# theori-io/nrsc5

Measured on AMD Instinct MI355X. Metric: IQ MS/s demod+decoded, higher is better.
Workload: dtype exact float32 half-band (== int16 Q15) / f32 OFDM + sync / int32 Viterbi metrics

## Files before the change

include/nrsc5hip.h:

```cpp
#ifndef NRSC5HIP_H_
#define NRSC5HIP_H_

#include <stddef.h>
#include <stdint.h>

#ifdef __cplusplus
extern "C" {
#endif

#define NRSC5HIP_OK            0
#define NRSC5HIP_EINVAL       (-1)
#define NRSC5HIP_ENOMEM       (-2)
#define NRSC5HIP_EHIP         (-3)
#define NRSC5HIP_EOVERFLOW    (-4)

#define NRSC5HIP_P1_FRAME_BITS   146176
#define NRSC5HIP_P1_FRAME_WORDS  4568
#define NRSC5HIP_PIDS_FRAME_BITS 80

enum { NRSC5HIP_MODE_FM = 0, NRSC5HIP_MODE_AM = 1 };
#define NRSC5HIP_AM_P1_FRAME_BITS  3750
#define NRSC5HIP_AM_P3_BITS_MA1    24000
#define NRSC5HIP_AM_P3_BITS_MA3    30000

// ... 33 lines not shown
    int32_t bc_decoded;
    uint32_t pids[3];
    uint32_t sis;
} nrsc5hip_record;

typedef struct nrsc5hip_config {
    int device;
    int max_streams;
    long long q15_capacity;
    int record_capacity;
    int p1_slots;
    int p1_async;
    int l2_feedback;
    int am_enable;
    int batch_zero_copy;
    int l2_index;
} nrsc5hip_config;

typedef struct nrsc5hip_engine nrsc5hip_engine;

int nrsc5hip_engine_create(const nrsc5hip_config *cfg, nrsc5hip_engine **out);
void nrsc5hip_engine_destroy(nrsc5hip_engine *e);
const char *nrsc5hip_last_error(void);
const char *nrsc5hip_source_sha(void);
void *nrsc5hip_engine_hip_stream(nrsc5hip_engine *e);

int nrsc5hip_device_count(int *n);
int nrsc5hip_device_upload(int device, const void *host, size_t nbytes, void **dev_out);
int nrsc5hip_device_free(int device, void *dev);

int nrsc5hip_push_cu8(nrsc5hip_engine *e, int stream, const uint8_t *iq, uint32_t nbytes);
int nrsc5hip_push_cs16(nrsc5hip_engine *e, int stream, const int16_t *iq, uint32_t n);
int nrsc5hip_stream_reset(nrsc5hip_engine *e, int stream);
#define NRSC5HIP_ABI_VERSION 16
int nrsc5hip_abi_version(void);
int nrsc5hip_stream_fresh(nrsc5hip_engine *e, int stream);
int nrsc5hip_stream_set_mode(nrsc5hip_engine *e, int stream, int mode);
int nrsc5hip_force_resync(nrsc5hip_engine *e, int stream);
long long nrsc5hip_bytes_to_next_block(nrsc5hip_engine *e, int stream, int cu8);
int nrsc5hip_drain_ready(nrsc5hip_engine *e, int stream, nrsc5hip_record *out, int max, int *n_out);
int nrsc5hip_stream_set_manual_step(nrsc5hip_engine *e, int stream, int on);
int nrsc5hip_stream_step(nrsc5hip_engine *e, int stream);
int nrsc5hip_stream_step_ahead(nrsc5hip_engine *e, int stream, int *submitted);

int nrsc5hip_batch_append_cu8(nrsc5hip_engine *e, int nstreams, const int *stream_ids,
                              const uint8_t *dev_iq, long long stride_bytes, const uint32_t *nbytes);
int nrsc5hip_batch_append_cs16(nrsc5hip_engine *e, int nstreams, const int *stream_ids,
                               const int16_t *dev_iq, long long stride_elems, const uint32_t *nelems);
#define NRSC5HIP_TRIM_RETAIN_MAX    ((8LL * 16 + 1) * 71280)
#define NRSC5HIP_TRIM_RETAIN_MAX_AM ((8LL * 8 + 1) * 8910)
int nrsc5hip_batch_trim(nrsc5hip_engine *e, int nstreams, const int *stream_ids, long long *retained);
int nrsc5hip_batch_process(nrsc5hip_engine *e, int nstreams, const int *stream_ids, int max_steps, int *steps_done);

int nrsc5hip_drain(nrsc5hip_engine *e, int stream, nrsc5hip_record *out, int max, int *n_out);
int nrsc5hip_p1_frame_packed(nrsc5hip_engine *e, int stream, int slot, uint32_t *words );
int nrsc5hip_p1_frame_bits(nrsc5hip_engine *e, int stream, int slot, uint8_t *bits );
int nrsc5hip_px_frame_bits(nrsc5hip_engine *e, int stream, int slot, int channel, int nbits, uint8_t *bits);
int nrsc5hip_batch_fetch_px(nrsc5hip_engine *e, int nstreams, const int *stream_ids, uint32_t *frames);
int nrsc5hip_am_frame_bits(nrsc5hip_engine *e, int stream, int slot, int which, int nbits, uint8_t *bits);
int nrsc5hip_batch_fetch(nrsc5hip_engine *e, int nstreams, const int *stream_ids, nrsc5hip_record *records,
                         int max_records, int *counts, uint32_t *frames);
int nrsc5hip_batch_fetch_view(nrsc5hip_engine *e, int nstreams, const nrsc5hip_record **records, int *counts, const uint32_t **frames);
void nrsc5hip_unpack_bits(const uint32_t *words, int nbits, uint8_t *bits);

#define NRSC5HIP_L2_MAX_PDUS     16
#define NRSC5HIP_L2_MAX_PACKETS  64
#define NRSC5HIP_L2_MAX_BYTES    18269
// ... 131 lines not shown
int nrsc5hip_stage_aas(nrsc5hip_aas *a, int nstreams, const int *targets, const uint8_t *const *packets, const int *nbytes,
                       nrsc5hip_aas_event_cb cb, void *opaque);
int nrsc5hip_stage_aas_frames(nrsc5hip_aas *a, nrsc5hip_psd *psd, nrsc5hip_engine *e, int nstreams, const int *targets, const uint8_t *const *bits,
                              const int *nbits, const int *nframes, const int *lcs, const int *reset_at, nrsc5hip_aas_event_cb cb, void *opaque);
int nrsc5hip_aas_debug_arena(nrsc5hip_aas *a, long long bytes);

int nrsc5hip_stage_halfband_fm_cu8(nrsc5hip_engine *e, const uint8_t *iq, uint32_t nbytes, int16_t *out );
int nrsc5hip_stage_fft2048(nrsc5hip_engine *e, const float *in , float *out, int n);
int nrsc5hip_stage_viterbi_k7(nrsc5hip_engine *e, const int8_t *soft , int len, int nframes,
                              uint8_t *bits );
int nrsc5hip_stage_first_header(nrsc5hip_engine *e, const uint8_t *bits, int nbits, int nframes, int threads, int *ok);
int nrsc5hip_stage_viterbi_k9(nrsc5hip_engine *e, const int8_t *soft , int len, int nframes,
                              const unsigned gens[3], uint8_t *bits );
int nrsc5hip_stage_selftest(nrsc5hip_engine *e, int *failures);
enum { NRSC5HIP_MATH_REF_SINCOSF = 0, NRSC5HIP_MATH_REF_ATAN2F, NRSC5HIP_MATH_FAST_SINCOS, NRSC5HIP_MATH_FAST_SINCOS_REDUCED,
       NRSC5HIP_MATH_FAST_ATAN2, NRSC5HIP_MATH_SMALL_COS_SIN, NRSC5HIP_MATH_SMALL_ATAN };
int nrsc5hip_stage_math(nrsc5hip_engine *e, int fn, const void *a, const void *b, long long n, void *out0, void *out1);
enum { NRSC5HIP_HB_ACQ = 0, NRSC5HIP_HB_SYM128, NRSC5HIP_HB_SYM256 };
int nrsc5hip_stage_halfband_raw(nrsc5hip_engine *e, int form, const uint8_t *iq, size_t nbytes, int lead, long long a0, long long n,
                                int16_t *out, uint32_t *probe);
int nrsc5hip_stage_p1_deint(nrsc5hip_engine *e, const int8_t *pm, uint32_t *out);
int nrsc5hip_stage_p1_frame(nrsc5hip_engine *e, const int8_t *soft, int walk, uint8_t *bits, int *errors);
int nrsc5hip_stage_pids(nrsc5hip_engine *e, const int8_t *pm, int bc, int8_t *coded, uint8_t *bits, int *crc_ok);
int nrsc5hip_stage_px_interleave(nrsc5hip_engine *e, int len, int npairs, const int8_t *pairs, int8_t *out, int *ready);
int nrsc5hip_stage_am_deinterleave(nrsc5hip_engine *e, int psmi, int nframes, const uint8_t *sym, int8_t *v1, int8_t *v3);
enum { NRSC5HIP_CODE_E1 = 1, NRSC5HIP_CODE_E2 = 2 };
int nrsc5hip_stage_am_epilogue(nrsc5hip_engine *e, const int8_t *soft, const uint8_t *bits, int len, int code, int threads, int *errors,
                               uint8_t *bits_out, uint32_t *words_out);
int nrsc5hip_stage_acquire(nrsc5hip_engine *e, int n, const int16_t *win, const int16_t *hist, const int *state, const int *fill,
                           int16_t *filt, float *sums, int *samperr, float *peak, int16_t *hist_out);
int nrsc5hip_stage_acquire_raw(nrsc5hip_engine *e, int n, const uint8_t *iq, long long nbytes, const long long *rd, const int16_t *hist, const int *state,
                               int16_t *acq_win, int16_t *filt, float *sums, int *samperr, float *peak, int16_t *hist_out);
int nrsc5hip_stage_am_acquire(nrsc5hip_engine *e, const int16_t *win, const int16_t *hist, int state, int fill, int *samperr, float *peak, int16_t *hist_out);
int nrsc5hip_stage_viterbi_k7_debug(nrsc5hip_engine *e, const int8_t *soft, int len, uint8_t *bits, unsigned long long *dec_out);
int nrsc5hip_stage_viterbi_bench(nrsc5hip_engine *e, int len, int nframes, int phases, int reps, float *ms_per_launch);
int nrsc5hip_stage_viterbi_k9_bench(nrsc5hip_engine *e, int len, int nframes, int phases, int reps, float *ms_per_launch);
enum {
    NRSC5HIP_TUNE_DECODE_STREAMS = 0,
    NRSC5HIP_TUNE_AM_DECODE_STREAMS,
    NRSC5HIP_TUNE_VERDICT_LAG,
    NRSC5HIP_TUNE_SYNC_PHASES,
    NRSC5HIP_TUNE_FWD_SEGMENTS
    , NRSC5HIP_TUNE_FWD_WARM
    , NRSC5HIP_TUNE_AM_SEGMENTS
    , NRSC5HIP_TUNE_DECODE_CUS
    , NRSC5HIP_TUNE_DECODE_PRIORITY
    , NRSC5HIP_TUNE_AM_WARM
    , NRSC5HIP_TUNE_MIXFFT_SYMS
    , NRSC5HIP_TUNE_DEFER_WAIT
    , NRSC5HIP_TUNE_TRACEBACK_WALK
    , NRSC5HIP_TUNE_SYNC_LANES
    , NRSC5HIP_TUNE_DIRECT_DECIMATE
    , NRSC5HIP_TUNE_EARLY_FLUSH_KB
    , NRSC5HIP_TUNE_SEAM_PREPARE
    , NRSC5HIP_TUNE_NCO_EXACT
    , NRSC5HIP_TUNE_FLOW_MIN
    , NRSC5HIP_TUNE_LOOP_EXACT
    , NRSC5HIP_TUNE_HOST_CAPTURE
    , NRSC5HIP_TUNE_FOLD_REPORT
};
void nrsc5hip_debug_seam_totals(double out[8], int reset);
void nrsc5hip_debug_seam_counts(double out[6], int reset);
int nrsc5hip_debug_poison_results(nrsc5hip_engine *e);
int nrsc5hip_debug_fwd_stats(nrsc5hip_engine *e, int stats[2]);
int nrsc5hip_debug_flow_stats(nrsc5hip_engine *e, long long stats[2]);
int nrsc5hip_debug_host_capture_stats(nrsc5hip_engine *e, long long stats[5]);
// ... 95 lines not shown
```

nrsc5_amd/csrc/engine_stage.hip:

```cpp
#include <algorithm>
#include <cmath>
#include "engine_internal.h"

extern "C" void nrsc5hip_debug_seam_totals(double out[8], int reset)
{
    for (int k = 0; k < 8; k++) { if (out) out[k] = g_seam[k]; if (reset) g_seam[k] = 0; }
}
extern "C" void nrsc5hip_debug_seam_counts(double out[6], int reset)
{
    for (int k = 0; k < 6; k++) { if (out) out[k] = g_seam[8 + k]; if (reset) g_seam[8 + k] = 0; }
}

extern "C" int nrsc5hip_stage_l2_index(nrsc5hip_engine *e, const uint8_t *bits, int nbits, int nframes, nrsc5hip_l2_frame *out, uint8_t *pdu_bytes, long long stride)
{
    ON_ENGINE_DEVICE(e);
    if (!e || !bits || !out || nbits < 1 || nframes < 1) FAIL(NRSC5HIP_EINVAL, "bad argument");
    const int words = (nbits + 31) / 32;
    std::vector<uint32_t> w((size_t)words * nframes, 0u);
    for (int f = 0; f < nframes; f++)
        for (int i = 0; i < nbits; i++) w[(size_t)f * words + (i >> 5)] |= (uint32_t)(bits[(size_t)f * nbits + i] & 1u) << (i & 31);
    DevTmp tw;
    HIPCHK(hipMalloc(&tw.p, w.size() * sizeof(uint32_t)));
    uint32_t *dw = (uint32_t *)tw.p;
    HIPCHK(hipMemcpy(dw, w.data(), w.size() * sizeof(uint32_t), hipMemcpyHostToDevice));
// ... 490 lines not shown
    std::vector<unsigned> counts((size_t)n, (unsigned)nbytes);
    HIPCHK(hipMemcpy(e->nbytes_dev, counts.data(), counts.size() * sizeof(unsigned), hipMemcpyHostToDevice));
    launch_attach_raw(e->db, n, nullptr, (const uint8_t *)draw.p, nbytes, e->nbytes_dev, e->main);
    HIPCHK(hipGetLastError());
    HIPCHK(hipStreamSynchronize(e->main));
    for (int s = 0; s < n; s++) {
        POKE(e->db.state + s, StreamState, rd, rd[s]);
        if ((rc = acq_poke(e, s, hist + (size_t)s * 62, state[s]))) return rc;
    }
    return acq_run_fm(e, n, acq_win, filt, sums, samperr, peak, hist_out);
}

extern "C" int nrsc5hip_stage_am_acquire(nrsc5hip_engine *e, const int16_t *win, const int16_t *hist, int state, int fill, int *samperr, float *peak, int16_t *hist_out)
{
    ON_ENGINE_DEVICE(e);
    if (!win || !hist || !samperr || !peak || !hist_out) FAIL(NRSC5HIP_EINVAL, "null argument");
    if (!e->db.am) FAIL(NRSC5HIP_EINVAL, "engine was created without am_enable");
    int rc = acq_check_common(e, 1, &state, MODE_AM, AM_WIN); if (rc) return rc;
    if (fill < 0 || fill > AM_WIN) FAIL(NRSC5HIP_EINVAL, "fill %d: 0 .. %d samples", fill, AM_WIN);
    if ((rc = nrsc5hip_stream_fresh(e, 0))) return rc;
    DevBuffers db = e->db;
    db.l2_ring = nullptr; db.l2_px_ring = nullptr; db.l2_am_ring = nullptr; db.p1_mirror = nullptr;
    HIPCHK(hipMemcpy(db.q15, win, (size_t)AM_WIN * sizeof(c16), hipMemcpyHostToDevice));
    POKE(db.state, StreamState, wr, (long long)fill);
    if ((rc = acq_poke(e, 0, hist, state))) return rc;
    HIPCHK(hipMemsetAsync(db.counters, 0, 4 * sizeof(int), e->main));
    launch_am_step(e->tb, db, 1, nullptr, e->main, e->cfg.l2_feedback, e->cfg.p1_async ? 0 : -1, 0, 0);
    HIPCHK(hipGetLastError());
    HIPCHK(hipStreamSynchronize(e->main));
    if ((rc = acq_peek(e, 0, samperr, peak, hist_out))) return rc;
    return nrsc5hip_stream_fresh(e, 0);
}

extern "C" int nrsc5hip_stage_viterbi_k7_debug(nrsc5hip_engine *e, const int8_t *soft, int len, uint8_t *bits, unsigned long long *dec_out)
{
    ON_ENGINE_DEVICE(e);
    if (!e || !soft || !bits || !dec_out || len < 64) FAIL(NRSC5HIP_EINVAL, "bad argument");
    int8_t *dsoft = nullptr; unsigned long long *ddec = nullptr; uint32_t *dout = nullptr;
    const int words = (len + 31) / 32;
    HIPCHK(hipMalloc((void **)&dsoft, (size_t)3 * len));
    HIPCHK(hipMalloc((void **)&ddec, (size_t)(len + 64) * sizeof(unsigned long long)));
    HIPCHK(hipMalloc((void **)&dout, (size_t)words * sizeof(uint32_t)));
    HIPCHK(hipMemcpy(dsoft, soft, (size_t)3 * len, hipMemcpyHostToDevice));
    if (launch_viterbi_frames(e->vit_scratch, dsoft, len, 1, ddec, dout, e->main)) FAIL(NRSC5HIP_EINVAL, "frame length %d not supported or out of device memory", len);
    HIPCHK(hipStreamSynchronize(e->main));
    std::vector<uint32_t> w(words);
    HIPCHK(hipMemcpy(w.data(), dout, w.size() * sizeof(uint32_t), hipMemcpyDeviceToHost));
    HIPCHK(hipMemcpy(dec_out, ddec, (size_t)(len + 64) * sizeof(unsigned long long), hipMemcpyDeviceToHost));
    nrsc5hip_unpack_bits(w.data(), len, bits);
    (void)hipFree(dsoft); (void)hipFree(ddec); (void)hipFree(dout);
    return 0;
}

extern "C" int nrsc5hip_stage_viterbi_bench(nrsc5hip_engine *e, int len, int nframes, int phases, int reps, float *ms_per_launch)
{
    ON_ENGINE_DEVICE(e);
    if (!e || !ms_per_launch || len < 64 || nframes < 1 || reps < 1) FAIL(NRSC5HIP_EINVAL, "bad argument");
    int8_t *dsoft = nullptr; unsigned long long *ddec = nullptr; uint32_t *dout = nullptr;
    const int words = (len + 31) / 32;
    std::vector<int8_t> h((size_t)nframes * 3 * len);
    unsigned x = 12345;
    for (auto &v : h) { x = x * 1664525u + 1013904223u; v = (int8_t)((int)(x >> 24) - 128); if (v == -128) v = -127; }
    HIPCHK(hipMalloc((void **)&dsoft, h.size()));
    HIPCHK(hipMalloc((void **)&ddec, (size_t)nframes * (len + 64) * sizeof(unsigned long long)));
    HIPCHK(hipMalloc((void **)&dout, (size_t)nframes * words * sizeof(uint32_t)));
    HIPCHK(hipMemcpy(dsoft, h.data(), h.size(), hipMemcpyHostToDevice));
// ... 198 lines not shown
```

nrsc5_amd/csrc/k_mixfft.hip:

```cpp
#include <hip/hip_runtime.h>
#include "kernels.h"
#include "wave_ops.h"
#include "fastmath.h"
#include "halfband_raw.h"
#include "prepare_block.h"

#include "mixfft_body.h"

namespace nrsc5 {

template <int SPW, int NPAR>
__global__ __launch_bounds__(128 * NPAR) MIXFFT_OCCUPANCY void k_mixfft(DevTables tb, DevBuffers db, const int *ids, int local_prepare)
{
    wave_set_priority_high();
    const int s = wave_uniform(stream_of(ids, blockIdx.y));
    __shared__ __attribute__((aligned(16))) uint8_t lds[sizeof(MixLds<NPAR>)];
    mixfft_wg<SPW, NPAR>(lds, tb, db, s, (int)blockIdx.x, local_prepare);
}

constexpr int P8_ROW = 288;
constexpr int P8_K2 = 36;
constexpr int TW8_N = 224;

template <int M> __device__ __forceinline__ cf cf_lane_xor(cf v)
// ... 207 lines not shown
#define MIXFFT8_OCCUPANCY
#endif
__global__ __launch_bounds__(256) MIXFFT8_OCCUPANCY void k_mixfft8(DevTables tb, DevBuffers db, const int *ids, int local_prepare)
{
    wave_set_priority_high();
    const int s = wave_uniform(stream_of(ids, blockIdx.y));
    const StreamState &st = db.state[s];
    SymParams sp;
    if (local_prepare) {
        __shared__ SymParams sh_sp;
        if (threadIdx.x == 0) {
            const Prepared p = prepare_values(st, false);
            sh_sp.active = p.active; sh_sp.a00 = (st.rd - st.base) + p.samperr; sh_sp.dtheta = p.dtheta; sh_sp.theta = p.theta; sh_sp.growth = p.growth; sh_sp.nco_mode = 0;
        }
        __syncthreads();
        sp = sh_sp;
    } else {
        sp.active = st.active; sp.a00 = (st.rd - st.base) + st.samperr_cur; sp.dtheta = st.dtheta; sp.theta = st.theta; sp.growth = st.growth; sp.nco_mode = st.nco_mode;
    }
    sp.active = wave_uniform(sp.active); sp.a00 = uniform64(sp.a00); sp.dtheta = uniform64(sp.dtheta); sp.theta = uniform64(sp.theta); sp.growth = uniform64(sp.growth); sp.nco_mode = wave_uniform(sp.nco_mode);
    if (!sp.active) return;
    __shared__ cf lds[8 * P8_ROW];
    static_assert(8 * P8_ROW >= 9 * 256 && 9 * 240 == SYM_N, "nine decimated samples per work-item fit in the FFT tile");
    __shared__ cf twB[TW8_N];
    if (sp.nco_mode) {
        if (st.raw) mixfft_symbol8<true, true>(tb, db, st, sp, s, lds, twB);
        else mixfft_symbol8<false, true>(tb, db, st, sp, s, lds, twB);
        return;
    }
    if (st.raw) mixfft_symbol8<true>(tb, db, st, sp, s, lds, twB);
    else mixfft_symbol8<false>(tb, db, st, sp, s, lds, twB);
}

__global__ __launch_bounds__(64) void k_nco_exact(DevBuffers db, const int *ids, int nstreams)
{
    const int idx = blockIdx.x;
    if (idx >= nstreams || threadIdx.x != 0) return;
    const int s = stream_of(ids, idx);
    StreamState &st = db.state[s];
    if (!st.active || !st.nco_mode) return;
    float pr = st.nco_re, pi = st.nco_im;
    const float c = st.inc_re, d = st.inc_im;
    float2 *tab = db.nco_tab + (size_t)s * NSYM * SYM_N;
    for (int sym = 0; sym < NSYM; sym++) {
#ifdef HIPEMU
        for (int j = 0; j < SYM_N; j++) {
            tab[sym * SYM_N + j] = make_float2(pr, pi);
            const float ac = pr * c, bd = pi * d, ad = pr * d, bc = pi * c;
            pr = ac - bd; pi = ad + bc;
        }
#else
        cf P = cf_make(pr, pi);
        const cf K = cf_make(c, d);
        cf *out = (cf *)(tab + sym * SYM_N);
#pragma unroll 8
        for (int j = 0; j < SYM_N; j++) {
            out[j] = P;
            cf t1, t2;
            asm("v_pk_mul_f32 %1, %0, %3 op_sel_hi:[0,1]\n\t"
                "v_pk_mul_f32 %2, %0, %3 op_sel:[1,1] op_sel_hi:[1,0]\n\t"
                "v_pk_add_f32 %0, %1, %2 neg_lo:[0,1]" : "+v"(P), "=&v"(t1), "=&v"(t2) : "v"(K));
        }
        pr = P.x; pi = P.y;
#endif
        const float m = (float)sqrt((double)pr * (double)pr + (double)pi * (double)pi);
        pr = pr / m; pi = pi / m;
    }
    st.nco_re = pr; st.nco_im = pi;
}

void launch_nco_exact(const DevBuffers &db, int nstreams, const int *stream_ids, hipStream_t st)
{
    if (!db.nco_tab) return;
    hipLaunchKernelGGL(k_nco_exact, dim3(nstreams), dim3(64), 0, st, db, stream_ids, nstreams);
}

void launch_mixfft(const DevTables &tb, const DevBuffers &db, int nstreams, const int *stream_ids, hipStream_t st, int syms_per_wg, int local_prepare)
{
    if (syms_per_wg == 32) { hipLaunchKernelGGL(k_mixfft8, dim3(NSYM, nstreams), dim3(256), 0, st, tb, db, stream_ids, local_prepare); return; }
    if (syms_per_wg == 16) { hipLaunchKernelGGL((k_mixfft<1, 2>), dim3(NSYM / 2, nstreams), dim3(256), 0, st, tb, db, stream_ids, local_prepare); return; }
    switch (syms_per_wg) {
    case 2: hipLaunchKernelGGL((k_mixfft<2, 1>), dim3(NSYM / 2, nstreams), dim3(128), 0, st, tb, db, stream_ids, local_prepare); break;
    case 4: hipLaunchKernelGGL((k_mixfft<4, 1>), dim3(NSYM / 4, nstreams), dim3(128), 0, st, tb, db, stream_ids, local_prepare); break;
    case 8: hipLaunchKernelGGL((k_mixfft<8, 1>), dim3(NSYM / 8, nstreams), dim3(128), 0, st, tb, db, stream_ids, local_prepare); break;
    default: hipLaunchKernelGGL((k_mixfft<1, 1>), dim3(NSYM, nstreams), dim3(128), syms_per_wg >= 100 ? (size_t)(syms_per_wg - 100) << 10 : 0, st, tb, db, stream_ids, local_prepare); break;
    }
}

__global__ __launch_bounds__(128) void k_fft2048(DevTables tb, const float2 *in, float2 *out)
{
    __shared__ cf lds[8 * PITCH_A];
    const int tid = threadIdx.x;
    const cf *src = (const cf *)(in + (size_t)blockIdx.x * FFT_N);
    cf *dst = (cf *)(out + (size_t)blockIdx.x * FFT_N);
    cf x[16];
#pragma unroll
    for (int h = 0; h < 2; h++)
#pragma unroll
        for (int n1 = 0; n1 < 8; n1++) x[8 * h + n1] = src[tid + 128 * h + 256 * n1];
    __shared__ cf twB[256];
    fft_stage_b_twiddles<128>(twB, tb.twiddle);
// ... 85 lines not shown
```

nrsc5_amd/engine.py:

```python
from __future__ import annotations

import ctypes
import os
import numpy as np

_HERE = os.path.dirname(os.path.abspath(__file__))
DEFAULT_LIB = os.path.join(_HERE, "libnrsc5hip.so")
_AB_LIB = os.environ.get("NRSC5HIP_AB_LIB")
if _AB_LIB:
    import sys as _sys
    print(f"nrsc5_amd.engine: NRSC5HIP_AB_LIB={_AB_LIB}: running a library that is NOT built from this tree (A/B measurement)", file=_sys.stderr)
    DEFAULT_LIB = _AB_LIB

from .abi import *
from .abi import _Config, _ChanConfig, _ScanConfig, _FmConfig
from .consumers import (HdcConsumer, PsdConsumer, SisConsumer, feed_hdc, feed_hdc_batch, feed_psd_batch, feed_sis_batch,
                        sis_utf8, sis_text, _sis_device_info, sis_event_fields, AasConsumer, feed_aas_batch, aas_event_fields, aas_sig_table, aas_packets)


def l2_frame_to_dict(fr: L2Frame) -> dict:
    out = {k: int(getattr(fr, k)) for k in ("pci", "nbytes", "n_pdu", "status", "end_offset", "lost_sync")}
    out["pdus"] = []
    for i in range(min(fr.n_pdu, 16)):
        p = fr.pdu[i]
# ... 36 lines not shown
    lib.nrsc5hip_drain.argtypes = [vp, ci, vp, ci, ctypes.POINTER(ci)]
    lib.nrsc5hip_p1_frame_packed.argtypes = [vp, ci, ci, vp]
    lib.nrsc5hip_p1_frame_bits.argtypes = [vp, ci, ci, vp]
    lib.nrsc5hip_batch_fetch.argtypes = [vp, ci, vp, vp, ci, vp, vp]
    lib.nrsc5hip_unpack_bits.argtypes = [vp, ci, vp]
    lib.nrsc5hip_unpack_bits.restype = None
    lib.nrsc5hip_stage_halfband_fm_cu8.argtypes = [vp, vp, ctypes.c_uint32, vp]
    lib.nrsc5hip_stage_fft2048.argtypes = [vp, vp, vp, ci]
    lib.nrsc5hip_stage_viterbi_k7.argtypes = [vp, vp, ci, ci, vp]
    lib.nrsc5hip_debug_fetch.argtypes = [vp, ci, vp, vp]
    lib.nrsc5hip_debug_fetch_costas.argtypes = [vp, ci, vp, vp]
    lib.nrsc5hip_stage_selftest.argtypes = [vp, ctypes.POINTER(ci)]
    lib.nrsc5hip_stage_viterbi_k7_debug.argtypes = [vp, vp, ci, vp, vp]
    lib.nrsc5hip_stage_viterbi_bench.argtypes = [vp, ci, ci, ci, ci, ctypes.POINTER(ctypes.c_float)]
    lib.nrsc5hip_debug_sync_phases.argtypes = [vp, vp]
    lib.nrsc5hip_debug_tune.argtypes = [vp, ci, ci]
    lib.nrsc5hip_debug_fwd_stats.argtypes = [vp, vp]
    lib.nrsc5hip_debug_flow_stats.argtypes = [vp, vp]
    lib.nrsc5hip_debug_host_capture_stats.argtypes = [vp, vp]
    lib.nrsc5hip_debug_k9_stats.argtypes = [vp, vp]
    lib.nrsc5hip_debug_tb_stats.argtypes = [vp, vp]
    lib.nrsc5hip_stage_first_header.argtypes = [vp, vp, ci, ci, ci, vp]
    lib.nrsc5hip_stage_math.argtypes = [vp, ci, vp, vp, ctypes.c_longlong, vp, vp]
    lib.nrsc5hip_stage_halfband_raw.argtypes = [vp, ci, vp, ctypes.c_size_t, ci, ctypes.c_longlong, ctypes.c_longlong, vp, vp]
    lib.nrsc5hip_stage_p1_deint.argtypes = [vp, vp, vp]
    lib.nrsc5hip_stage_p1_frame.argtypes = [vp, vp, ci, vp, vp]
    lib.nrsc5hip_stage_pids.argtypes = [vp, vp, ci, vp, vp, vp]
    lib.nrsc5hip_stage_px_interleave.argtypes = [vp, ci, ci, vp, vp, vp]
    lib.nrsc5hip_stage_am_deinterleave.argtypes = [vp, ci, ci, vp, vp, vp]
    lib.nrsc5hip_stage_am_epilogue.argtypes = [vp, vp, vp, ci, ci, ci, vp, vp, vp]
    lib.nrsc5hip_stage_acquire.argtypes = [vp, ci, vp, vp, vp, vp, vp, vp, vp, vp, vp]
    lib.nrsc5hip_stage_acquire_raw.argtypes = [vp, ci, vp, ctypes.c_longlong, vp, vp, vp, vp, vp, vp, vp, vp, vp]
    lib.nrsc5hip_stage_am_acquire.argtypes = [vp, vp, vp, ci, ci, vp, vp, vp]
    lib.nrsc5hip_debug_poison_results.argtypes = [vp]
    lib.nrsc5hip_debug_seam_totals.argtypes = [vp, ci]
    lib.nrsc5hip_debug_seam_totals.restype = None
    lib.nrsc5hip_debug_seam_counts.argtypes = [vp, ci]
    lib.nrsc5hip_debug_seam_counts.restype = None
    lib.nrsc5hip_drain_ready.argtypes = [vp, ci, vp, ci, ctypes.POINTER(ci)]
    lib.nrsc5hip_stream_set_manual_step.argtypes = [vp, ci, ci]
    lib.nrsc5hip_stream_step.argtypes = [vp, ci]
    lib.nrsc5hip_stream_step_ahead.argtypes = [vp, ci, ctypes.POINTER(ci)]
    lib.nrsc5hip_batch_fetch_view.argtypes = [vp, ci, ctypes.POINTER(vp), vp, ctypes.POINTER(vp)]
    lib.nrsc5hip_reset_all.argtypes = [vp]
    lib.nrsc5hip_profile.argtypes = [vp, ci, vp, vp]
    lib.nrsc5hip_l2_index.argtypes = [vp, ci, vp, vp, vp, ctypes.c_longlong]
    lib.nrsc5hip_stage_l2_index.argtypes = [vp, vp, ci, ci, vp, vp, ctypes.c_longlong]
    lib.nrsc5hip_l2_frame_get.argtypes = [vp, ci, ci, vp]
    lib.nrsc5hip_batch_fetch_l2.argtypes = [vp, ci, vp, vp]
    lib.nrsc5hip_batch_fetch_l2_px.argtypes = [vp, ci, vp, vp]
    lib.nrsc5hip_batch_fetch_l2_am.argtypes = [vp, ci, vp, vp]
    lib.nrsc5hip_hdc_create.argtypes = [ci, ctypes.POINTER(vp)]
    lib.nrsc5hip_hdc_destroy.argtypes = [vp]
    lib.nrsc5hip_hdc_destroy.restype = None
    lib.nrsc5hip_hdc_reset.argtypes = [vp, ci]
    lib.nrsc5hip_hdc_push_frame.argtypes = [vp, ci, ci, vp, vp]
    lib.nrsc5hip_hdc_fixed_audio_end.argtypes = [vp, ci, ci, vp, ctypes.c_uint]
    lib.nrsc5hip_hdc_fixed_audio_end.restype = ctypes.c_uint
    lib.nrsc5hip_l2_apply_audio_end.argtypes = [vp, ctypes.c_uint]
    lib.nrsc5hip_hdc_frame_reset.argtypes = [vp, ci]
    lib.nrsc5hip_hdc_advance.argtypes = [vp, ci, ci, HDC_CB, vp]
    lib.nrsc5hip_hdc_adts.argtypes = [vp, ctypes.c_uint, vp]
    lib.nrsc5hip_hdc_adts.restype = ctypes.c_size_t
    lib.nrsc5hip_hdc_host_bytes.argtypes = [vp]
    lib.nrsc5hip_hdc_host_bytes.restype = ctypes.c_size_t
    lib.nrsc5hip_hdc_feed.argtypes = [vp, vp, ci, vp, vp, vp, vp, ci, HDC_CB, vp]
# ... 37 lines not shown
    lib.nrsc5hip_chan_clip_counts.argtypes = [vp, vp]
    lib.nrsc5hip_chan_feed.argtypes = [vp, vp, vp, vp, ll]
    lib.nrsc5hip_chan_feed_fm.argtypes = [vp, vp, vp, vp, vp, ll, vp, ll, ll, ctypes.POINTER(ll)]
    lib.nrsc5hip_fm_create.argtypes = [ctypes.POINTER(_FmConfig), ctypes.POINTER(vp)]
    lib.nrsc5hip_fm_destroy.argtypes = [vp]
    lib.nrsc5hip_fm_destroy.restype = None
    lib.nrsc5hip_fm_reset.argtypes = [vp]
    lib.nrsc5hip_fm_info.argtypes = [vp, ctypes.POINTER(ci), ctypes.POINTER(ci), ctypes.POINTER(ci), ctypes.POINTER(ll)]
    lib.nrsc5hip_fm_taps.argtypes = [vp, vp, vp]
    lib.nrsc5hip_fm_outputs_for.argtypes = [vp, ll]
    lib.nrsc5hip_fm_outputs_for.restype = ll
    lib.nrsc5hip_fm_process.argtypes = [vp, vp, ll, ll, vp, ll, ll, ctypes.POINTER(ll)]
    lib.nrsc5hip_fm_clip_counts.argtypes = [vp, vp]
    lib.nrsc5hip_fm_pilot.argtypes = [vp, vp, vp]
    lib.nrsc5hip_stage_fm_mpx.argtypes = [vp, vp, ll, ll, vp, vp]
    lib.nrsc5hip_scan_create.argtypes = [ctypes.POINTER(_ScanConfig), ctypes.POINTER(vp)]
    lib.nrsc5hip_scan_destroy.argtypes = [vp]
    lib.nrsc5hip_scan_destroy.restype = None
    lib.nrsc5hip_scan_reset.argtypes = [vp]
    lib.nrsc5hip_scan_push.argtypes = [vp, vp, ll]
    lib.nrsc5hip_scan_info.argtypes = [vp, ctypes.POINTER(ci), ctypes.POINTER(ll), ctypes.POINTER(ctypes.c_double)]
    lib.nrsc5hip_scan_spectrum.argtypes = [vp, vp]
    lib.nrsc5hip_scan_detect.argtypes = [vp, ctypes.POINTER(ScanParams), vp, ci, ctypes.POINTER(ci)]
    lib.nrsc5hip_scan_detect_psd.argtypes = [vp, ci, ctypes.c_double, ctypes.POINTER(ScanParams), vp, ci, ctypes.POINTER(ci)]
    return lib


EXPORTED_SYMBOLS = [
    "nrsc5hip_engine_create", "nrsc5hip_engine_destroy", "nrsc5hip_last_error", "nrsc5hip_source_sha", "nrsc5hip_engine_hip_stream",
    "nrsc5hip_push_cu8", "nrsc5hip_push_cs16", "nrsc5hip_stream_reset", "nrsc5hip_stream_fresh", "nrsc5hip_force_resync", "nrsc5hip_bytes_to_next_block",
    "nrsc5hip_batch_append_cu8", "nrsc5hip_batch_append_cs16", "nrsc5hip_batch_process", "nrsc5hip_batch_trim", "nrsc5hip_drain",
    "nrsc5hip_p1_frame_packed", "nrsc5hip_p1_frame_bits", "nrsc5hip_batch_fetch", "nrsc5hip_unpack_bits",
    "nrsc5hip_stage_halfband_fm_cu8", "nrsc5hip_stage_fft2048", "nrsc5hip_stage_viterbi_k7", "nrsc5hip_debug_fetch", "nrsc5hip_debug_fetch_costas",
    "nrsc5hip_debug_fetch_q15", "nrsc5hip_debug_alloc_copy", "nrsc5hip_debug_free", "nrsc5hip_reset_all", "nrsc5hip_profile", "nrsc5hip_stage_selftest", "nrsc5hip_stage_viterbi_k7_debug", "nrsc5hip_stage_viterbi_bench", "nrsc5hip_debug_sync_phases", "nrsc5hip_debug_tune", "nrsc5hip_debug_fwd_stats", "nrsc5hip_debug_flow_stats", "nrsc5hip_debug_host_capture_stats", "nrsc5hip_abi_version", "nrsc5hip_debug_tb_stats", "nrsc5hip_debug_k9_stats", "nrsc5hip_stage_first_header", "nrsc5hip_stage_math", "nrsc5hip_stage_halfband_raw", "nrsc5hip_stage_p1_deint", "nrsc5hip_stage_p1_frame", "nrsc5hip_stage_pids", "nrsc5hip_stage_px_interleave", "nrsc5hip_stage_am_deinterleave", "nrsc5hip_stage_am_epilogue", "nrsc5hip_stage_acquire", "nrsc5hip_stage_acquire_raw", "nrsc5hip_stage_am_acquire", "nrsc5hip_debug_seam_totals", "nrsc5hip_debug_seam_counts", "nrsc5hip_drain_ready", "nrsc5hip_stream_set_manual_step", "nrsc5hip_stream_step", "nrsc5hip_stream_step_ahead", "nrsc5hip_debug_poison_results", "nrsc5hip_device_count", "nrsc5hip_device_upload", "nrsc5hip_device_free", "nrsc5hip_batch_fetch_view", "nrsc5hip_batch_fetch_l2_px", "nrsc5hip_batch_fetch_l2_am",
    "nrsc5hip_stream_set_mode", "nrsc5hip_am_frame_bits", "nrsc5hip_stage_viterbi_k9", "nrsc5hip_px_frame_bits",
    "nrsc5hip_batch_fetch_px", "nrsc5hip_debug_fetch_px", "nrsc5hip_stage_viterbi_k9_bench",
    "nrsc5hip_l2_index", "nrsc5hip_stage_l2_index", "nrsc5hip_l2_frame_get", "nrsc5hip_batch_fetch_l2",
    "nrsc5hip_hdc_create", "nrsc5hip_hdc_destroy", "nrsc5hip_hdc_reset", "nrsc5hip_hdc_push_frame", "nrsc5hip_hdc_advance",
    "nrsc5hip_hdc_adts", "nrsc5hip_hdc_host_bytes", "nrsc5hip_hdc_fixed_audio_end", "nrsc5hip_l2_apply_audio_end", "nrsc5hip_hdc_frame_reset",
    "nrsc5hip_hdc_feed",
    "nrsc5hip_psd_create", "nrsc5hip_psd_destroy", "nrsc5hip_psd_reset", "nrsc5hip_psd_feed", "nrsc5hip_psd_stats", "nrsc5hip_stage_psd", "nrsc5hip_stage_psd_streams",
    "nrsc5hip_sis_create", "nrsc5hip_sis_destroy", "nrsc5hip_sis_reset", "nrsc5hip_sis_feed", "nrsc5hip_sis_get", "nrsc5hip_sis_stats", "nrsc5hip_stage_sis",
    "nrsc5hip_sis_debug_arena",
    "nrsc5hip_aas_create", "nrsc5hip_aas_destroy", "nrsc5hip_aas_reset", "nrsc5hip_aas_feed", "nrsc5hip_aas_stats", "nrsc5hip_aas_sig", "nrsc5hip_stage_aas",
    "nrsc5hip_stage_aas_frames", "nrsc5hip_aas_debug_arena",
    "nrsc5hip_chan_create", "nrsc5hip_chan_destroy", "nrsc5hip_chan_reset", "nrsc5hip_chan_info", "nrsc5hip_chan_taps",
    "nrsc5hip_chan_outputs_for", "nrsc5hip_chan_process", "nrsc5hip_chan_clip_counts", "nrsc5hip_chan_feed",
    "nrsc5hip_scan_create", "nrsc5hip_scan_destroy", "nrsc5hip_scan_reset", "nrsc5hip_scan_push", "nrsc5hip_scan_info",
    "nrsc5hip_scan_spectrum", "nrsc5hip_scan_detect", "nrsc5hip_scan_detect_psd",
    "nrsc5hip_fm_create", "nrsc5hip_fm_destroy", "nrsc5hip_fm_reset", "nrsc5hip_fm_info", "nrsc5hip_fm_taps", "nrsc5hip_fm_outputs_for",
    "nrsc5hip_fm_process", "nrsc5hip_fm_clip_counts", "nrsc5hip_fm_pilot", "nrsc5hip_stage_fm_mpx", "nrsc5hip_chan_feed_fm"]


def library_sha(path: str | None = None) -> str:
    path = path or DEFAULT_LIB
    if not os.path.exists(path):
        raise Nrsc5HipError(f"{path} not found: build it with `python -m nrsc5_amd.build` (hipcc, gfx950). There is no CPU fallback.")
    data = open(path, "rb").read()
    marker = b"NRSC5HIP_SOURCE_SHA="
    k = data.find(marker)
    if k < 0:
        return "unmarked"
    return data[k + len(marker):k + len(marker) + 16].split(b"\0")[0].decode(errors="replace")


def check_fresh(path: str | None = None):
    from . import build
# ... 407 lines not shown
        if raw:
            out["acq_win"] = np.zeros((n, ACQ_WIN_FM, 2), dtype=np.int16)
        return out

    def stage_acquire(self, win, hist, state, fill, n: int | None = None) -> dict:
        n = len(state) if n is None else n
        m = max(n, 0)
        win, hist = _exact(win, np.int16, m * ACQ_WIN_FM * 2), _exact(hist, np.int16, m * 62)
        state, fill = _exact(state, np.int32, m), _exact(fill, np.int32, m)
        o = self._acq_outputs(n)
        self._check(self.lib.nrsc5hip_stage_acquire(self._h, n, _ptr(win), _ptr(hist), _ptr(state), _ptr(fill), o["filt"].ctypes.data, o["sums"].ctypes.data,
                                                    o["samperr"].ctypes.data, o["peak"].ctypes.data, o["hist_out"].ctypes.data))
        return o

    def stage_acquire_raw(self, iq, rd, hist, state, n: int | None = None) -> dict:
        n = len(state) if n is None else n
        m = max(n, 0)
        nbytes = 0
        if iq is not None:
            iq = np.ascontiguousarray(iq, dtype=np.uint8)
            nbytes = iq.size // max(m, 1)
            iq = iq.reshape(-1)
        rd, hist, state = _exact(rd, np.int64, m), _exact(hist, np.int16, m * 62), _exact(state, np.int32, m)
        o = self._acq_outputs(n, raw=True)
        self._check(self.lib.nrsc5hip_stage_acquire_raw(self._h, n, _ptr(iq), nbytes, _ptr(rd), _ptr(hist), _ptr(state), o["acq_win"].ctypes.data, o["filt"].ctypes.data,
                                                        o["sums"].ctypes.data, o["samperr"].ctypes.data, o["peak"].ctypes.data, o["hist_out"].ctypes.data))
        return o

    def stage_am_acquire(self, win, hist, state: int, fill: int = ACQ_WIN_AM) -> dict:
        win, hist = _exact(win, np.int16, ACQ_WIN_AM * 2), _exact(hist, np.int16, 62)
        se, peak, hist_out = ctypes.c_int(0), np.zeros(2, dtype=np.float32), np.zeros((31, 2), dtype=np.int16)
        self._check(self.lib.nrsc5hip_stage_am_acquire(self._h, _ptr(win), _ptr(hist), state, fill, ctypes.byref(se), peak.ctypes.data, hist_out.ctypes.data))
        return dict(samperr=np.array([se.value], dtype=np.int32), peak=peak[None], hist_out=hist_out[None])

    def stage_selftest(self) -> int:
        n = ctypes.c_int(-1)
        self._check(self.lib.nrsc5hip_stage_selftest(self._h, ctypes.byref(n)))
        return n.value

    def debug_fetch_costas(self, stream: int):
        f = np.zeros(534, dtype=np.float32); p = np.zeros(534, dtype=np.float32)
        self._check(self.lib.nrsc5hip_debug_fetch_costas(self._h, stream, f.ctypes.data, p.ctypes.data))
        return f, p

    def debug_fetch_px(self, stream: int) -> np.ndarray:
        out = np.zeros((2, 2, 4608), dtype=np.int8)
        self.lib.nrsc5hip_debug_fetch_px.argtypes = [ctypes.c_void_p, ctypes.c_int, ctypes.c_void_p]
        self._check(self.lib.nrsc5hip_debug_fetch_px(self._h, stream, out.ctypes.data))
        return out

    def debug_fetch(self, stream: int):
        pm = np.zeros(16 * 23040, dtype=np.int8)
        bins = np.zeros((32, 534), dtype=np.complex64)
        self._check(self.lib.nrsc5hip_debug_fetch(self._h, stream, pm.ctypes.data, bins.ctypes.data))
        return pm, bins


class Channelizer:

    OUT_RATE = 744187.5

    def __init__(self, rate, fmt: int, offsets_hz, gains=None, device: int = 0, lib_path: str | None = None):
        from fractions import Fraction
        self.lib = load_library(lib_path)
        r = Fraction(rate).limit_denominator(1 << 20) if isinstance(rate, float) else Fraction(rate)
        self.rate_num, self.rate_den = r.numerator, r.denominator
# ... 335 lines not shown
```

Before: 275,700.

## Spread the exact NCO recurrence across a wavefront with exec-mask shifting

The exact oscillator table kernel previously ran one thread per stream, writing each symbol's samples one at a time. It now uses all 64 lanes: the recurrence still runs serially, but through an inline-asm .rept loop that shifts the exec mask left by one bit before each step, so each lane holds a distinct step's value. Stores then become one coalesced row of 64, and the running phasor is broadcast from the last lane with readlane. The goal is to keep the bit-exact sequential multiply chain while replacing 2160 scalar stores per symbol with wide coalesced writes. The exec-mask manipulation in inline asm is fragile, and a stage test entry point is added to check it.

Result: faster. 281,800, median of 6 (+2.2%).

```diff
diff --git a/include/nrsc5hip.h b/include/nrsc5hip.h
--- a/include/nrsc5hip.h
+++ b/include/nrsc5hip.h
@@ -89,7 +89,7 @@
 int nrsc5hip_push_cu8(nrsc5hip_engine *e, int stream, const uint8_t *iq, uint32_t nbytes);
 int nrsc5hip_push_cs16(nrsc5hip_engine *e, int stream, const int16_t *iq, uint32_t n);
 int nrsc5hip_stream_reset(nrsc5hip_engine *e, int stream);
-#define NRSC5HIP_ABI_VERSION 16
+#define NRSC5HIP_ABI_VERSION 17
 int nrsc5hip_abi_version(void);
 int nrsc5hip_stream_fresh(nrsc5hip_engine *e, int stream);
 int nrsc5hip_stream_set_mode(nrsc5hip_engine *e, int stream, int mode);
@@ -287,6 +287,7 @@
 int nrsc5hip_stage_acquire_raw(nrsc5hip_engine *e, int n, const uint8_t *iq, long long nbytes, const long long *rd, const int16_t *hist, const int *state,
                                int16_t *acq_win, int16_t *filt, float *sums, int *samperr, float *peak, int16_t *hist_out);
 int nrsc5hip_stage_am_acquire(nrsc5hip_engine *e, const int16_t *win, const int16_t *hist, int state, int fill, int *samperr, float *peak, int16_t *hist_out);
+int nrsc5hip_stage_nco_exact(nrsc5hip_engine *e, int n, const float *start, const float *inc, const int *active, const int *nco_mode, float *tab, float *end);
 int nrsc5hip_stage_viterbi_k7_debug(nrsc5hip_engine *e, const int8_t *soft, int len, uint8_t *bits, unsigned long long *dec_out);
 int nrsc5hip_stage_viterbi_bench(nrsc5hip_engine *e, int len, int nframes, int phases, int reps, float *ms_per_launch);
 int nrsc5hip_stage_viterbi_k9_bench(nrsc5hip_engine *e, int len, int nframes, int phases, int reps, float *ms_per_launch);
diff --git a/nrsc5_amd/csrc/engine_stage.hip b/nrsc5_amd/csrc/engine_stage.hip
--- a/nrsc5_amd/csrc/engine_stage.hip
+++ b/nrsc5_amd/csrc/engine_stage.hip
@@ -546,6 +546,37 @@
     return nrsc5hip_stream_fresh(e, 0);
 }
 
+extern "C" int nrsc5hip_stage_nco_exact(nrsc5hip_engine *e, int n, const float *start, const float *inc, const int *active, const int *nco_mode, float *tab, float *end)
+{
+    ON_ENGINE_DEVICE(e);
+    if (!start || !inc || !active || !nco_mode || !tab || !end) FAIL(NRSC5HIP_EINVAL, "null argument");
+    if (n < 1 || n > e->cfg.max_streams) FAIL(NRSC5HIP_EINVAL, "%d streams: 1 .. max_streams (%d)", n, e->cfg.max_streams);
+    if (!e->db.nco_tab) FAIL(NRSC5HIP_EINVAL, "the engine has no oscillator table");
+    int rc;
+    for (int s = 0; s < n; s++) {
+        if (e->mode_host[s] != MODE_FM) FAIL(NRSC5HIP_EINVAL, "stream %d must be in FM mode", s);
+        if ((rc = nrsc5hip_stream_fresh(e, s))) return rc;
+    }
+    const size_t row = (size_t)NSYM * SYM_N;
+    HIPCHK(hipMemset(e->db.nco_tab, ACQ_FILL, (size_t)n * row * sizeof(float2)));
+    for (int s = 0; s < n; s++) {
+        POKE(e->db.state + s, StreamState, active, active[s] ? 1 : 0);
+        POKE(e->db.state + s, StreamState, nco_mode, nco_mode[s] ? 1 : 0);
+        POKE(e->db.state + s, StreamState, nco_re, start[2 * s]);
+        POKE(e->db.state + s, StreamState, nco_im, start[2 * s + 1]);
+        POKE(e->db.state + s, StreamState, inc_re, inc[2 * s]);
+        POKE(e->db.state + s, StreamState, inc_im, inc[2 * s + 1]);
+    }
+    launch_nco_exact(e->db, n, nullptr, e->main);
+    HIPCHK(hipGetLastError());
+    HIPCHK(hipStreamSynchronize(e->main));
+    HIPCHK(hipMemcpy(tab, e->db.nco_tab, (size_t)n * row * sizeof(float2), hipMemcpyDeviceToHost));
+    static_assert(offsetof(StreamState, nco_im) - offsetof(StreamState, nco_re) == 4, "nco_re, nco_im are adjacent words");
+    for (int s = 0; s < n; s++) HIPCHK(hipMemcpy(end + 2 * s, (const char *)(e->db.state + s) + offsetof(StreamState, nco_re), 2 * sizeof(float), hipMemcpyDeviceToHost));
+    for (int s = 0; s < n; s++) if ((rc = nrsc5hip_stream_fresh(e, s))) return rc;
+    return 0;
+}
+
 extern "C" int nrsc5hip_stage_viterbi_k7_debug(nrsc5hip_engine *e, const int8_t *soft, int len, uint8_t *bits, unsigned long long *dec_out)
 {
     ON_ENGINE_DEVICE(e);
diff --git a/nrsc5_amd/csrc/k_mixfft.hip b/nrsc5_amd/csrc/k_mixfft.hip
--- a/nrsc5_amd/csrc/k_mixfft.hip
+++ b/nrsc5_amd/csrc/k_mixfft.hip
@@ -263,10 +263,28 @@
     else mixfft_symbol8<false>(tb, db, st, sp, s, lds, twB);
 }
 
+#ifndef HIPEMU
+#define NCO_STEP "v_pk_mul_f32 %[t1], %[p], %[k] op_sel_hi:[0,1]\n\tv_pk_mul_f32 %[t2], %[p], %[k] op_sel:[1,1] op_sel_hi:[1,0]\n\t"
+#define NCO_ADD "v_pk_add_f32 %[p], %[t1], %[t2] neg_lo:[0,1]"
+template <int R> __device__ __forceinline__ cf nco_row(cf &P, const cf K)
+{
+    cf t1, t2;
+    asm volatile(".rept %c[n]\n\ts_lshl_b64 exec, exec, 1\n\t" NCO_STEP NCO_ADD "\n\t.endr\n\ts_mov_b64 exec, -1"
+                 : [p] "+v"(P), [t1] "=&v"(t1), [t2] "=&v"(t2) : [k] "v"(K), [n] "n"(R - 1) : "scc");
+    const cf mine = P;
+    const float lx = mine.x, ly = mine.y;
+    P = cf_make(__int_as_float(__builtin_amdgcn_readlane(__float_as_int(lx), R - 1)), __int_as_float(__builtin_amdgcn_readlane(__float_as_int(ly), R - 1)));
+    asm(NCO_STEP NCO_ADD : [p] "+v"(P), [t1] "=&v"(t1), [t2] "=&v"(t2) : [k] "v"(K));
+    return mine;
+}
+#endif
 __global__ __launch_bounds__(64) void k_nco_exact(DevBuffers db, const int *ids, int nstreams)
 {
     const int idx = blockIdx.x;
-    if (idx >= nstreams || threadIdx.x != 0) return;
+    if (idx >= nstreams) return;
+#ifdef HIPEMU
+    if (threadIdx.x != 0) return;
+#endif
     const int s = stream_of(ids, idx);
     StreamState &st = db.state[s];
     if (!st.active || !st.nco_mode) return;
@@ -281,23 +299,21 @@
             pr = ac - bd; pi = ad + bc;
         }
 #else
+        constexpr int ROWS = SYM_N / 64, TAIL = SYM_N % 64;
+        static_assert(ROWS * 64 + TAIL == SYM_N && TAIL > 0, "a symbol is whole rows of 64 steps and a shorter tail");
+        const int lane = threadIdx.x;
         cf P = cf_make(pr, pi);
         const cf K = cf_make(c, d);
         cf *out = (cf *)(tab + sym * SYM_N);
-#pragma unroll 8
-        for (int j = 0; j < SYM_N; j++) {
-            out[j] = P;
-            cf t1, t2;
-            asm("v_pk_mul_f32 %1, %0, %3 op_sel_hi:[0,1]\n\t"
-                "v_pk_mul_f32 %2, %0, %3 op_sel:[1,1] op_sel_hi:[1,0]\n\t"
-                "v_pk_add_f32 %0, %1, %2 neg_lo:[0,1]" : "+v"(P), "=&v"(t1), "=&v"(t2) : "v"(K));
-        }
+        for (int row = 0; row < ROWS; row++) { const cf mine = nco_row<64>(P, K); out[row * 64 + lane] = mine; }
+        const cf mine = nco_row<TAIL>(P, K);
+        if (lane < TAIL) out[ROWS * 64 + lane] = mine;
         pr = P.x; pi = P.y;
 #endif
         const float m = (float)sqrt((double)pr * (double)pr + (double)pi * (double)pi);
         pr = pr / m; pi = pi / m;
     }
-    st.nco_re = pr; st.nco_im = pi;
+    if (threadIdx.x == 0) { st.nco_re = pr; st.nco_im = pi; }
 }
 
 void launch_nco_exact(const DevBuffers &db, int nstreams, const int *stream_ids, hipStream_t st)
diff --git a/nrsc5_amd/engine.py b/nrsc5_amd/engine.py
--- a/nrsc5_amd/engine.py
+++ b/nrsc5_amd/engine.py
@@ -92,6 +92,7 @@
     lib.nrsc5hip_stage_acquire.argtypes = [vp, ci, vp, vp, vp, vp, vp, vp, vp, vp, vp]
     lib.nrsc5hip_stage_acquire_raw.argtypes = [vp, ci, vp, ctypes.c_longlong, vp, vp, vp, vp, vp, vp, vp, vp, vp]
     lib.nrsc5hip_stage_am_acquire.argtypes = [vp, vp, vp, ci, ci, vp, vp, vp]
+    lib.nrsc5hip_stage_nco_exact.argtypes = [vp, ci, vp, vp, vp, vp, vp, vp]
     lib.nrsc5hip_debug_poison_results.argtypes = [vp]
     lib.nrsc5hip_debug_seam_totals.argtypes = [vp, ci]
     lib.nrsc5hip_debug_seam_totals.restype = None
@@ -195,7 +196,7 @@
     "nrsc5hip_batch_append_cu8", "nrsc5hip_batch_append_cs16", "nrsc5hip_batch_process", "nrsc5hip_batch_trim", "nrsc5hip_drain",
     "nrsc5hip_p1_frame_packed", "nrsc5hip_p1_frame_bits", "nrsc5hip_batch_fetch", "nrsc5hip_unpack_bits",
     "nrsc5hip_stage_halfband_fm_cu8", "nrsc5hip_stage_fft2048", "nrsc5hip_stage_viterbi_k7", "nrsc5hip_debug_fetch", "nrsc5hip_debug_fetch_costas",
-    "nrsc5hip_debug_fetch_q15", "nrsc5hip_debug_alloc_copy", "nrsc5hip_debug_free", "nrsc5hip_reset_all", "nrsc5hip_profile", "nrsc5hip_stage_selftest", "nrsc5hip_stage_viterbi_k7_debug", "nrsc5hip_stage_viterbi_bench", "nrsc5hip_debug_sync_phases", "nrsc5hip_debug_tune", "nrsc5hip_debug_fwd_stats", "nrsc5hip_debug_flow_stats", "nrsc5hip_debug_host_capture_stats", "nrsc5hip_abi_version", "nrsc5hip_debug_tb_stats", "nrsc5hip_debug_k9_stats", "nrsc5hip_stage_first_header", "nrsc5hip_stage_math", "nrsc5hip_stage_halfband_raw", "nrsc5hip_stage_p1_deint", "nrsc5hip_stage_p1_frame", "nrsc5hip_stage_pids", "nrsc5hip_stage_px_interleave", "nrsc5hip_stage_am_deinterleave", "nrsc5hip_stage_am_epilogue", "nrsc5hip_stage_acquire", "nrsc5hip_stage_acquire_raw", "nrsc5hip_stage_am_acquire", "nrsc5hip_debug_seam_totals", "nrsc5hip_debug_seam_counts", "nrsc5hip_drain_ready", "nrsc5hip_stream_set_manual_step", "nrsc5hip_stream_step", "nrsc5hip_stream_step_ahead", "nrsc5hip_debug_poison_results", "nrsc5hip_device_count", "nrsc5hip_device_upload", "nrsc5hip_device_free", "nrsc5hip_batch_fetch_view", "nrsc5hip_batch_fetch_l2_px", "nrsc5hip_batch_fetch_l2_am",
+    "nrsc5hip_debug_fetch_q15", "nrsc5hip_debug_alloc_copy", "nrsc5hip_debug_free", "nrsc5hip_reset_all", "nrsc5hip_profile", "nrsc5hip_stage_selftest", "nrsc5hip_stage_viterbi_k7_debug", "nrsc5hip_stage_viterbi_bench", "nrsc5hip_debug_sync_phases", "nrsc5hip_debug_tune", "nrsc5hip_debug_fwd_stats", "nrsc5hip_debug_flow_stats", "nrsc5hip_debug_host_capture_stats", "nrsc5hip_abi_version", "nrsc5hip_debug_tb_stats", "nrsc5hip_debug_k9_stats", "nrsc5hip_stage_first_header", "nrsc5hip_stage_math", "nrsc5hip_stage_halfband_raw", "nrsc5hip_stage_p1_deint", "nrsc5hip_stage_p1_frame", "nrsc5hip_stage_pids", "nrsc5hip_stage_px_interleave", "nrsc5hip_stage_am_deinterleave", "nrsc5hip_stage_am_epilogue", "nrsc5hip_stage_acquire", "nrsc5hip_stage_acquire_raw", "nrsc5hip_stage_am_acquire", "nrsc5hip_stage_nco_exact", "nrsc5hip_debug_seam_totals", "nrsc5hip_debug_seam_counts", "nrsc5hip_drain_ready", "nrsc5hip_stream_set_manual_step", "nrsc5hip_stream_step", "nrsc5hip_stream_step_ahead", "nrsc5hip_debug_poison_results", "nrsc5hip_device_count", "nrsc5hip_device_upload", "nrsc5hip_device_free", "nrsc5hip_batch_fetch_view", "nrsc5hip_batch_fetch_l2_px", "nrsc5hip_batch_fetch_l2_am",
     "nrsc5hip_stream_set_mode", "nrsc5hip_am_frame_bits", "nrsc5hip_stage_viterbi_k9", "nrsc5hip_px_frame_bits",
     "nrsc5hip_batch_fetch_px", "nrsc5hip_debug_fetch_px", "nrsc5hip_stage_viterbi_k9_bench",
     "nrsc5hip_l2_index", "nrsc5hip_stage_l2_index", "nrsc5hip_l2_frame_get", "nrsc5hip_batch_fetch_l2",
@@ -669,6 +670,15 @@
         se, peak, hist_out = ctypes.c_int(0), np.zeros(2, dtype=np.float32), np.zeros((31, 2), dtype=np.int16)
         self._check(self.lib.nrsc5hip_stage_am_acquire(self._h, _ptr(win), _ptr(hist), state, fill, ctypes.byref(se), peak.ctypes.data, hist_out.ctypes.data))
         return dict(samperr=np.array([se.value], dtype=np.int32), peak=peak[None], hist_out=hist_out[None])
+
+    def stage_nco_exact(self, start, inc, active, nco_mode, n: int | None = None):
+        n = len(active) if n is None else n
+        m = max(n, 0)
+        start, inc = _exact(start, np.float32, 2 * m), _exact(inc, np.float32, 2 * m)
+        active, nco_mode = _exact(active, np.int32, m), _exact(nco_mode, np.int32, m)
+        tab, end = np.zeros((m, 32 * 2160, 2), dtype=np.float32), np.zeros((m, 2), dtype=np.float32)
+        self._check(self.lib.nrsc5hip_stage_nco_exact(self._h, n, _ptr(start), _ptr(inc), _ptr(active), _ptr(nco_mode), tab.ctypes.data, end.ctypes.data))
+        return tab, end
 
     def stage_selftest(self) -> int:
         n = ctypes.c_int(-1)
```
